# agiger/GPR

Measured on AMD Instinct MI355X. Metric: GP fits/sec (kernel build + Cholesky + solve), N=16384 d=32 fp64, higher is better.
Workload: dtype f64

## Files before the change

### gpr_amd/csrc/gprx_api.cpp

```cpp
#include <hip/hip_runtime.h>
#include <rccl/rccl.h>

#include <algorithm>
#include <climits>
#include <chrono>
#include <cmath>
#include <cstdlib>
#include <cstring>
#include <limits>
#include <memory>
#include <mutex>
#include <string>
#include <type_traits>
#include <vector>

#include "gprx_dist.h"
#include "gprx_internal.h"
#include "../../include/gprx_dev.h"

namespace gprx {

template <typename T>
void launch_pair_kernel(const KCanon<T>& K, const T* Xa, const T* Xb, int64_t q, int d, T* out, hipStream_t s);
template <typename T>
// ... 771 lines not shown
    } else if (!direct_build && pairs_mma_supported<T>(K, 1)) {
        const int64_t kf = pairs_feature_cols<T>(K, M->d);
        M->featU.ensure(sizeof(T) * np * kf);
        M->featV.ensure(sizeof(T) * np * kf);
        launch_pair_features<T>(K, M->X.as<T>(), n, M->d, M->X.as<T>(), false, M->featU.as<T>(), np, s,
                                M->flag.as<int>());
        launch_pair_features<T>(K, M->X.as<T>(), n, M->d, M->X.as<T>(), true, M->featV.as<T>(), np, s);
        const KCanon<T>* kdev = M->kfit.put(K, s);
        if (!separate_build && potrf_uses_tiles())
            tb = pairs_tile_build<T>(K, kdev, M->featU.as<T>(), M->featV.as<T>(), np, M->d, n, sigma2,
                                     M->flag.as<int>());
        if (!tb.mode)
            launch_kbuild_mma<T>(K, kdev, M->featU.as<T>(), M->featV.as<T>(), np, M->d, M->A.as<T>(),
                                 ld, n, sigma2, M->flag.as<int>(), s);
        launch_aug_rows<T>(M->Y.as<T>(), n, M->m, M->A.as<T>(), ld, np, mp, s);
    } else {
        launch_kbuild<T>(K, M->X.as<T>(), M->tab.as<T>(), n, M->X.as<T>(), M->tab.as<T>(), n, M->d, M->A.as<T>(), ld,
                         np, true, sigma2, M->flag.as<int>(), s);
        launch_aug_rows<T>(M->Y.as<T>(), n, M->m, M->A.as<T>(), ld, np, mp, s);
    }
    GPRX_HIP(hipEventRecord(ctx->ev[1], s));
    if (tb.mode || want_inv) {
        potrf_tiles<T>(M->A.as<T>(), ld, np, ld, M->Linv.as<T>(), M->info.as<int>(), ctx->ex, tb.mode ? &tb : nullptr,
                       want_inv ? (int)(np / GT) : 0);
    } else {
        potrf_auto<T>(M->A.as<T>(), ld, np, ld, M->Linv.as<T>(), M->info.as<int>(), ctx->ex);
    }
    GPRX_HIP(hipEventRecord(ctx->ev[2], s));
    launch_fit_reductions<T>(M->A.as<T>(), ld, n, np, M->m, M->red.as<double>(), s);
    launch_backsolve_chain<T>(M->A.as<T>(), ld, np, M->m, M->Linv.as<T>(), M->alpha.as<T>(), M->info.as<int>(), ctx->ex,
                              s);
    if (want_inv) {
        M->C.ensure(sizeof(T) * np * np);
        const T* U = M->A.as<T>() + np + mp;
        launch_gemm_nt_kskip<T>(M->C.as<T>(), np, U, ld, U, ld, np, np, np, s);
    }
    GPRX_HIP(hipEventRecord(ctx->ev[3], s));
    M->hstat.ensure(4 * sizeof(double));
    volatile double* hs = static_cast<double*>(M->hstat.p);
    launch_fit_status_gather(M->flag.as<int>(), M->info.as<int>(), M->red.as<double>(), M->hstat.dev, s);
    GPRX_HIP(hipStreamSynchronize(s));
    GPRX_HIP(hipGetLastError());
    int hflag = 0, hinfo = 0;
    double hred[2] = {hs[2], hs[3]};
    hflag = reinterpret_cast<volatile int*>(hs)[0];
    hinfo = reinterpret_cast<volatile int*>(hs + 1)[0];
    M->fitted = false;
// ... 2062 lines not shown
```

### gpr_amd/csrc/gprx_dev.cpp

```cpp
#include <hip/hip_runtime.h>

#include <algorithm>
#include <climits>
#include <cstring>
#include <string>
#include <vector>

#include "../../include/gprx_dev.h"
#include "gprx_internal.h"

namespace gprx {
template <typename T>
void launch_gemm_nt(T* C, int64_t ldc, const T* A, int64_t lda, const T* B, int64_t ldb, int64_t M, int64_t N,
                    int64_t K, T alpha, T beta, bool lower, hipStream_t s);
template <typename T>
void launch_diag_public(T* Akk, int64_t ld, T* Lk, int* info, int64_t col0, hipStream_t s, int ph = 3);
template <typename T>
void launch_diag_prof(T* Akk, int64_t ld, T* Lk, int* info, long long* prof, hipStream_t s);
namespace pt {
template <typename T>
void launch_diag_bench(int variant, T* A, int64_t ld, T* Linv, int* info, long long* prof, int reps, hipStream_t s);
}
}

// ... 284 lines not shown
}
extern "C" int64_t gprx_dev_bs_trace(int64_t* times, int64_t max_blocks) {
    try {
        return gprx::bs_trace_copy((long long*)times, max_blocks);
    } catch (const Error& e) {
        std::fprintf(stderr, "gprx_dev_bs_trace: %s\n", e.msg.c_str());
        return -1;
    }
}
extern "C" int64_t gprx_dev_pt_trace(int32_t* tasks, int64_t* times, int64_t max) {
    try {
        return gprx::pt_trace_copy(tasks, (long long*)times, max);
    } catch (const gprx::Error& e) {
        std::fprintf(stderr, "gprx_dev_pt_trace: %s\n", e.msg.c_str());
        return -1;
    }
}
extern "C" int32_t gprx_dev_pt_debug(int32_t* out, int32_t max_wg) { return gprx::pt_debug_snapshot(out, max_wg); }

extern "C" gprx_status gprx_dev_schedule(int32_t nc, int32_t nr, int32_t P, int32_t build, double* est_us,
                                         int64_t* ntasks) {
    try {
        const int64_t n = potrf_tiles_schedule_stats(nc, nr, P, (build & 1) != 0, est_us, (build & 2) ? nc : 0,
                                                     ((build >> 8) & 0xff) - 1, nullptr, 0, ((build >> 16) & 0xff) - 1);
        if (ntasks) *ntasks = n;
        return GPRX_OK;
    } catch (const Error& e) {
        std::fprintf(stderr, "gprx_dev_schedule: %s\n", e.msg.c_str());
        return e.st;
    }
}

extern "C" int64_t gprx_dev_schedule_list(int32_t nc, int32_t nr, int32_t P, int32_t build, int32_t* out,
                                          int64_t max) {
    try {
        return potrf_tiles_schedule_stats(nc, nr, P, (build & 1) != 0, nullptr, (build & 2) ? nc : 0,
                                          ((build >> 8) & 0xff) - 1, out, max, ((build >> 16) & 0xff) - 1);
    } catch (const Error& e) {
        std::fprintf(stderr, "gprx_dev_schedule_list: %s\n", e.msg.c_str());
        return -1;
    }
}

namespace gprx {
gprx_status gprx_dev_bench_impl(gprx_dtype dtype, int32_t what, int64_t M, int64_t N, int64_t K, int32_t iters,
                                double* ms, Exec* ex) {
    return dtype == GPRX_F64 ? bench_impl<double>(what, M, N, K, iters, ms, *ex)
                             : bench_impl<float>(what, M, N, K, iters, ms, *ex);
}
}

extern "C" gprx_status gprx_dev_fexp(gprx_ctx* ctx, const double* x, int64_t n, double* y) {
    (void)ctx;
    if (n <= 0) return GPRX_OK;
    double *dx = nullptr, *dy = nullptr;
    if (hipMalloc(&dx, sizeof(double) * n) != hipSuccess || hipMalloc(&dy, sizeof(double) * n) != hipSuccess)
        return GPRX_ERR_OOM;
    (void)hipMemcpy(dx, x, sizeof(double) * n, hipMemcpyHostToDevice);
    hipLaunchKernelGGL(dev_fexp_kernel, dim3((unsigned)((n + 255) / 256)), dim3(256), 0, 0, dx, n, dy);
    const hipError_t e = hipMemcpy(y, dy, sizeof(double) * n, hipMemcpyDeviceToHost);
// ... 53 lines not shown
```

### gpr_amd/csrc/gprx_internal.h

```cpp
#pragma once

#include <hip/hip_runtime.h>
#include <rccl/rccl.h>
#include <cstdint>
#include <cstdio>
#include <string>
#include <vector>

#include "../../include/gprx.h"

namespace gprx {

constexpr int MAX_LEAF = 8;
constexpr int MAX_TERM = 16;
constexpr int MAX_PER = 2;

enum LeafType { L_GAUSS = 1, L_GAUSS_EXP = 2, L_WHITE = 3, L_RQ = 4, L_PERIODIC = 5 };

template <typename T>
struct KLeaf {
    int type;
    int pslot;
    T c0, c1, c2;
    T p[3];
// ... 394 lines not shown
                         double* acc, hipStream_t s,
                         const uint64_t* ctab = nullptr);
template <typename T>
void launch_lml_grad_mma_cross(const KCanon<T>& K, const KCanon<T>* Kd, const T* Xa, int64_t na, const T* Xb,
                               int64_t nb, const T* center, int d, const T* FU, int64_t nfu, const T* FV, int64_t nfv,
                               T* GU, T* GV, const T* a, const T* b, const T* C, int64_t ldc, double* part, double* acc,
                               hipStream_t s);
template <typename T>
void launch_lml_grad_cross(const KCanon<T>& K, const T* Xa, const T* tabA, int64_t na, const T* Xb, const T* tabB,
                           int64_t nb, int d, const T* a, const T* b, const T* C, int64_t ldc, double* acc,
                           hipStream_t s);
template <typename T>
void launch_sparse_resid(const T* A, int64_t lda, int64_t n, int64_t M, const T* u, const T* y, T alpha, T* out,
                         hipStream_t s);
template <typename T>
void launch_sq_sum(const T* y, int64_t n, double* out, hipStream_t s);
template <typename T>
void launch_sub(const T* X, const T* Y, T* Z, int64_t e, hipStream_t s);
template <typename T>
TileBuild<T> pairs_tile_build(const KCanon<T>& K, const KCanon<T>* Kd, const T* FU, const T* FV, int64_t nf, int d,
                              int64_t n, T sigma2, int* flag);
template <typename T>
void potrf_tiles(T* A, int64_t ld, int64_t np, int64_t nrows, T* Linv, int* info, Exec& ex,
                 const TileBuild<T>* build = nullptr, int ni = 0, bool build_only = false);
template <typename T>
void launch_gemm_nt_kskip(T* C, int64_t ldc, const T* A, int64_t lda, const T* B, int64_t ldb, int64_t M, int64_t N,
                          int64_t K, hipStream_t s);
template <typename T>
void potrf_auto(T* A, int64_t ld, int64_t np, int64_t nrows, T* Linv, int* info, Exec& ex);
bool potrf_uses_tiles();
int64_t potrf_tiles_schedule_stats(int nc, int nr, int P, bool build, double* est_us, int ni = 0, int ratio = -1,
                                   int32_t* list_out = nullptr, int64_t list_max = 0, int pair = -1);
template <typename T>
void launch_gemm_nt(T* C, int64_t ldc, const T* A, int64_t lda, const T* B, int64_t ldb, int64_t M, int64_t N,
                    int64_t K, T alpha, T beta, bool lower, hipStream_t s);
template <typename T>
void launch_gemm_nt_splitk(T* C, int64_t ldc, int64_t cstride, const T* A, int64_t lda, const T* B, int64_t ldb,
                           int64_t M, int64_t N, int64_t K, int P, T alpha, bool lower, hipStream_t s);

template <typename T>
void launch_syrk_splitk(T* C, int64_t ldc, int64_t cstride, const T* A, int64_t lda, int64_t M, int64_t N, int64_t K,
                        int P, T alpha, hipStream_t s);
template <typename T>
bool launch_gemm_tall(T* C, int64_t ldc, const T* A, int64_t lda, const T* B, int64_t ldb, int64_t M, int64_t N,
                      int64_t K, T alpha, T beta, hipStream_t s);

template <typename T>
void launch_backsolve(const T* A, int64_t ld, int64_t np, int m, const T* Linv, T* z, T* alpha, hipStream_t s);

constexpr long long CHAIN_TLIMIT_TICKS = 400000000LL;

struct BlockTrace {
    long long* dev = nullptr;
    int n = 0;
    long long* ensure(int nb) {
// ... 61 lines not shown
```

### gpr_amd/csrc/k_mma.h

```cpp
#pragma once
#include "gprx_internal.h"
#include "k_handoff.h"

namespace gprx {
namespace mm {

constexpr int NT = 512;
constexpr int PAD = 16;

enum { T_DIAGX = 0, T_TRSM = 1, T_UPD = 2, T_BUILD = 3, T_TPART = 4, T_UPD2 = 5 };
enum { C_TICKET = 0, C_ERR = 1, C_NCTL = 16 };

typedef double d4_t __attribute__((ext_vector_type(4)));
typedef float f4_t __attribute__((ext_vector_type(4)));
typedef double d2_t __attribute__((ext_vector_type(2)));

template <typename T>
struct Mfma;
template <>
struct Mfma<double> {
    typedef d4_t acc_t;
    typedef d2_t vec_t;
    static constexpr int VEC = 2;
    __device__ static inline acc_t mma(double a, double b, acc_t c) {
// ... 384 lines not shown
            const int kr = kq * 4 + lk;
            fa[r] = a[S::at(kr, 16 * w + lr)];
#pragma unroll
            for (int g = G0; g < 8; g++) fb[r][g] = b[S::at(kr, 16 * g + lr)];
        };
        frag(0, 0);
#pragma unroll
        for (int kq = 0; kq < BK / 4; kq++) {
            if (kq + 1 < BK / 4) frag(kq + 1, (kq + 1) & 1);
            __builtin_amdgcn_sched_barrier(0);
#pragma unroll
            for (int g = G0; g < 8; g++) acc[g >> 2][g & 3] = Tr::mma(fb[kq & 1][g], fa[kq & 1], acc[g >> 2][g & 3]);
        }
    };
    static_assert(NST <= 8, "trirows: at most 8 stages");
    stage(std::integral_constant<int, 0>{});
    if constexpr (NST > 1) stage(std::integral_constant<int, (NST > 1 ? 1 : 0)>{});
    if constexpr (NST > 2) stage(std::integral_constant<int, (NST > 2 ? 2 : 0)>{});
    if constexpr (NST > 3) stage(std::integral_constant<int, (NST > 3 ? 3 : 0)>{});
    if constexpr (NST > 4) stage(std::integral_constant<int, (NST > 4 ? 4 : 0)>{});
    if constexpr (NST > 5) stage(std::integral_constant<int, (NST > 5 ? 5 : 0)>{});
    if constexpr (NST > 6) stage(std::integral_constant<int, (NST > 6 ? 6 : 0)>{});
    if constexpr (NST > 7) stage(std::integral_constant<int, (NST > 7 ? 7 : 0)>{});
}

template <typename T>
constexpr size_t tall_lds() {
    return sizeof(T) * 2 * 3 * Stage<T>::GRP * Stage<T>::SRP;
}
template <typename T, int MID = 1>
__device__ __forceinline__ void tile_mma_tall(typename Mfma<T>::acc_t (&acc)[4][4], const T* __restrict__ A,
                                              int64_t lda, const T* __restrict__ B, int64_t ldb, int K, T* smem,
                                              const int t, const T* __restrict__ Csub = nullptr, int64_t ldc = 0) {
    typedef Mfma<T> Tr;
    typedef Stage<T> S;
    constexpr int BK = BkOf<T>::v;
    static_assert(S::ROT == 0, "tall tile: unrotated staging");
    constexpr int GR3 = 3 * S::GRP, IPW3 = GR3 / 8, STG3 = GR3 * S::SRP;
    static_assert(GR3 % 8 == 0, "tall tile: whole DMA instructions per wave");
    const int lane = t & 63, w = t >> 6;
    const int wr = w & 3, wc = w >> 2, lr = lane & 15, lk = lane >> 4;
    const int lcol = lane / S::LPC, lrow = S::src_row(lane);
    auto issue = [&](int st) {
        T* buf = smem + (st & 1) * STG3;
#pragma unroll
        for (int u = 0; u < IPW3; u++) {
// ... 203 lines not shown
```

### gpr_amd/csrc/k_ptiles.hip

```cpp
#include "gprx_dist.h"
#include "gprx_internal.h"
#include "k_handoff.h"
#include "k_pairs.h"

#include <algorithm>
#include <climits>
#include <cstring>
#include <cstdlib>
#include <functional>
#include <map>
#include <mutex>
#include <queue>
#include <tuple>

namespace gprx {

namespace pt {

using namespace mm;
using ho::ld_agent;
using ho::ld_sys;
using ho::ld_uni;
using ho::local_sync;
using ho::publish;
// ... 50 lines not shown
}

#ifndef GPRX_TRSM_ROWS
#define GPRX_TRSM_ROWS 1
#endif
template <typename T>
__device__ __forceinline__ void tile_trsm(T* C, int64_t ldc, const T* A, int64_t lda,
                                          const T* __restrict__ B, int64_t ldb, T* smem, const int t) {
    if constexpr (!GPRX_TRSM_ROWS) {
        tile_gemm<T, false, 1, GPRX_SHORT_FEED>(C, ldc, A, lda, B, ldb, GT, false, smem, t, true);
    } else {
        typedef Mfma<T> Tr;
        const int lane = t & 63, w = t >> 6, lr = lane & 15, lk = lane >> 4;
        typename Tr::acc_t acc[2][4];
        mm::tile_mma_trirows<T>(acc, A, lda, B, ldb, smem, t);
#pragma unroll
        for (int x = 0; x < 2; x++)
#pragma unroll
            for (int y = 0; y < 4; y++)
#pragma unroll
                for (int reg = 0; reg < 4; reg++)
                    st_sc1(C + (int64_t)(16 * (4 * x + y) + Tr::orow(lk, reg)) * ldc + 16 * w + lr, acc[x][y][reg]);
    }
}

template <typename T>
__device__ __forceinline__ void tile_gemm_tall(T* __restrict__ C, int64_t ldc, const T* __restrict__ A, int64_t lda,
                                               const T* __restrict__ B, int64_t ldb, int K, T* smem, const int t) {
    typedef Mfma<T> Tr;
    typedef typename Tr::acc_t acc_t;
    const int lane = t & 63, w = t >> 6;
    const int wr = w & 3, wc = w >> 2, lr = lane & 15, lk = lane >> 4;
    acc_t acc[4][4];
    mm::tile_mma_tall<T, 1>(acc, A, lda, B, ldb, K, smem, t, C, ldc);
#pragma unroll
    for (int x = 0; x < 4; x++)
#pragma unroll
        for (int reg = 0; reg < 4; reg++) {
            T* ccol = C + (int64_t)(64 * wc + 16 * x + Tr::orow(lk, reg)) * ldc;
#pragma unroll
            for (int y = 0; y < 4; y++) st_sc1(ccol + 64 * wr + 16 * y + lr, -acc[x][y][reg]);
        }
}

constexpr int SPL = DB + 4;
constexpr int SIL = DB + 2;
// ... 945 lines not shown
template <typename T>
struct Args {
    T* A;
    int64_t ld;
    T* Linv;
    const int4* tasks;
    int ntasks;
    int nc;
    int nv;
    int* ctl;
    int* lcnt;
    int* ver;
    int* info;
    long long tlimit;
    int* dbg;
    int variant;
    long long* trace;
    long long* xt;
    const TileBuild<T>* tb;
    const PtDist<T>* dist;
    int split;
    T* pbuf;
    int* tflag;
};


constexpr int DIST_TO_REC = 132;
__device__ __forceinline__ void dist_note_timeout(int* rec, int kind, int type, int i, int j, int b0nb, int detail,
                                                  int seen) {
    if (!rec) return;
    if (__hip_atomic_fetch_add(rec, 0, __ATOMIC_RELAXED, __HIP_MEMORY_SCOPE_AGENT) != 0) return;
    if (atomicCAS(rec, 0, kind) != 0) return;
    rec[1] = type;
    rec[2] = i;
    rec[3] = j;
    rec[4] = b0nb;
    rec[5] = detail;
    rec[6] = seen;
}

template <typename T>
__device__ __forceinline__ T* dist_tile(T* A, const PtDist<T>& D, int i, int j) {
    const int li = __builtin_amdgcn_readfirstlane(D.loc[i]);
    int col = j;
    if (i > D.nc) {
        const int aa = i - D.nc - 1;
        col = (j < D.nc) ? j - aa : D.nc - aa + (j - D.nc - 1);
// ... 1001 lines not shown
                    dist_push(Akm, D, cm & ~first, owin, dist_f_tile() + (int64_t)k * D.nc + (k - 1), tid, tix, tgv);
                if (ok) dist_push(a.Linv + (int64_t)k * DB * DB, D, all & ~first, olinv, dist_f_linv(D.nr, D.nc) + k, tid);
            }
            if (!ok) break;
        } else {
        T* Ci = a.A + (int64_t)i * GT;
        constexpr bool fused_ts = std::is_same<T, double>::value && DIAG_LA;
        if (type == T_TPART) {
            if constexpr (SPLIT_CODE)
                (void)tpart_task<T, false>(tpc, Ci + (int64_t)(i - 1) * GT * ld, Ci + (int64_t)i * GT * ld, ld,
                                           a.Linv + (int64_t)(i - 1) * DB * DB, i, j, smem, s_ok, tid,
                                           tp_linv_form() ? nullptr
                                                          : a.A + (int64_t)(i - 1) * GT + (int64_t)(i - 1) * GT * ld);
        } else if (type == T_BUILD) {
            const TileBuild<T>& b = *a.tb;
            const bool bad = pr::build_tile_sum<T, 1, true>(b.Kd, b.FU, b.FV, b.nf, b.Kr, b.Kp, b.hd, a.A, ld, b.n,
                                                            b.sigma2, (int64_t)i * GT, (int64_t)j * GT, smem, tid);
            if (__builtin_amdgcn_readfirstlane(__any(bad))) atomicOr(a.tb->flag, 1);
            publish(a.ver + (int64_t)i * a.nv + j, 0, false);
        } else if (type == T_UPD) {
            const int64_t oa = (a.variant & 64) ? 0 : (int64_t)i * GT + (int64_t)b0 * GT * ld;
            const int64_t ob = (a.variant & 64) ? GT : (int64_t)j * GT + (int64_t)b0 * GT * ld;
            const int64_t lop = (a.variant & 128) ? 0 : ld;
            if (!(a.variant & 2))
                tile_gemm<T, true>(Ci + (int64_t)j * GT * ld, ld, a.A + oa, lop, a.A + ob, lop, nb * GT, i == j, smem,
                                   tid);
            publish(a.ver + (int64_t)i * a.nv + j, b0 + nb, false);
        } else if (type == T_UPD2) {
            if (!(a.variant & 2))
                tile_gemm_tall<T>(Ci + (int64_t)j * GT * ld, ld, a.A + (int64_t)i * GT + (int64_t)b0 * GT * ld, ld,
                                  a.A + (int64_t)j * GT + (int64_t)b0 * GT * ld, ld, nb * GT, smem, tid);
            publish2(a.ver + (int64_t)i * a.nv + j, a.ver + (int64_t)(i + 1) * a.nv + j, b0 + nb);
        } else if (type == T_TRSM) {
            T* Cik = Ci + (int64_t)j * GT * ld;
            if (!(a.variant & 1))
                tile_trsm<T>(Cik, ld, Cik, ld, a.Linv + (int64_t)j * DB * DB, DB, smem, tid);
            publish(a.lcnt + i, j + 1, false);
        } else {
            const int k = i;
            T* Akk = Ci + (int64_t)k * GT * ld;
            long long dt[4] = {0, 0, 0, 0};
            if (SPLIT_CODE && k > 0 && a.split) {
                if constexpr (fused_ts) (void)diagx_split<T>(tpc, k, smem, s_ok, tid);
                else (void)diagx_split_wait<T>(tpc, k, s_ok);
                if (a.trace) dt[0] = dt[1] = wall_clock64();
            } else if (fused_ts && k > 0) {
                T* Akm = Ci + (int64_t)(k - 1) * GT * ld;
                dt[0] = diagx_ts<T>(Akm, Akk, ld, a.Linv + (int64_t)(k - 1) * DB * DB, a.lcnt + k, k, smem, tid,
                                    a.trace != nullptr);
// ... 27 lines not shown
            tp[3] = (long long)blockIdx.x | (((long long)__builtin_amdgcn_s_memtime() - tc1) << 16);
        }
    }
    dbg_mark(a.dbg, -1, 9, 0, 0);
    if (wv == 0 && ld_agent(a.ctl + C_ERR)) atomicMin(a.info, -1);
}

struct Cost {
    double k128 = 17.1;
    double ovh = 6.5;
    double trsm = 16.0;
    double diagx = 70.0;
    double diag0 = 40.0;
    double early = 31.0;
    double diagf = 0.97;
    double build = 28.0;
    double tpart = 11.5, tpart_c = 0.0;
    double diagx_s = 44.0, early_s = 2.0;
    double tpart_prog = 2.5;
    bool prog = false;
    int np = 4;
    double tall = 0.975;
    int pair_nbmin = 1, pair_tail = 0;
};

static void order_tparts(std::vector<int4>& list) {
    std::map<int, std::vector<int>> pos;
    for (size_t q = 0; q < list.size(); q++)
        if ((list[q].x & 0xff) == T_TPART) pos[list[q].y].push_back((int)q);
    for (auto& kv : pos) {
        std::vector<int>& v = kv.second;
        std::sort(v.begin(), v.end());
        for (size_t u = 0; u < v.size(); u++) list[v[u]].z = (int)v.size() - 1 - (int)u;
    }
}

struct Task {
    int type, i, j, b0, nb;
    double dur;
    std::vector<int> succ, esucc;
    int ndep = 0;
    double bl = 0;
};

struct Schedule {
    std::vector<int4> list;
// ... 14 lines not shown
                if (p == W && b % W) continue;
                const int end = b + p;
                if (end > e - near || p > ratio * (e - end)) continue;
                break;
            }
            out.push_back({s + b, p});
            b += p;
        }
        return;
    }
    int hb = std::max(0, std::min(W * ((j - s) / W), e));
    hb -= hb % W;
    int b = 0;
    for (; b + W <= hb; b += W) out.push_back({s + b, W});
    for (int p = W / 2; p >= 1; p /= 2)
        if (b + p <= e - near) {
            out.push_back({s + b, p});
            b += p;
        }
    for (; b < e; b++) out.push_back({s + b, 1});
}

static Schedule make_schedule(int nc, int nr, int W, int near, int P, const Cost& cm0, bool build, int ni = 0,
                              int ratio = 0, bool split = false, int tail = 0, int pair = 0) {
    Cost cm = cm0;
    if (split) cm.early = cm.early_s;
    const int nr0 = nr - ni;
    auto start_of = [&](int i) { return i >= nr0 ? i - nr0 : 0; };
    static const bool id_pair = [] {
        const char* e = std::getenv("GPRX_PT_IDPAIR");
        return !(e && std::atoi(e) == 0);
    }();
    const bool ident_even = id_pair && pair > 0 && ni > 1;
    static const bool id_tail = [] {
        const char* e = std::getenv("GPRX_PT_IDTAIL");
        return !(e && std::atoi(e) == 0);
    }();
    auto cstart = [&](int i) {
        const int a = start_of(i);
        return (ident_even && i >= nr0) ? a - (a & 1) : a;
    };
    auto pair_role = [&](int i, int j) {
        if (pair <= 0) return 0;
        if (i >= nr0) {
            const int a = i - nr0;
            if (!ident_even) return 0;
            if ((a & 1) == 0) return a + 1 < ni ? 1 : 0;
            return 2;
        }
        const int r0 = j + pair;
        if (i >= r0 && (i - r0) % 2 == 0 && i + 1 < nr0) return 1;
        if (i - 1 >= r0 && (i - 1 - r0) % 2 == 0) return 2;
        return 0;
    };
    std::vector<Task> tasks;
    tasks.reserve((size_t)nr * nc * 2);
    auto add = [&](int type, int i, int j, int b0, int nb, double dur) {
        Task tk;
        tk.type = type;
        tk.i = i;
        tk.j = j;
        tk.b0 = b0;
        tk.nb = nb;
        tk.dur = dur;
        tasks.push_back(std::move(tk));
        return (int)tasks.size() - 1;
    };
    std::vector<int> diagx(nc, -1);
    std::vector<int> trsm((size_t)nr * nc, -1);
    std::vector<int> last_upd((size_t)nr * nc, -1);
    std::vector<std::vector<int>> deps, edeps;
    auto dep = [&](int tsk, int on, bool early = false) {
        if (on < 0) return;
        auto& d = early ? edeps : deps;
        if ((int)d.size() <= tsk) d.resize(tsk + 1);
// ... 51 lines not shown
            if (k < start_of(i)) continue;
            const int id = add(T_TRSM, i, k, 0, 0, cm.trsm);
            trsm[(size_t)i * nc + k] = id;
            dep(id, diagx[k]);
            dep(id, last_upd[(size_t)i * nc + k]);
        }
        if (k + 1 < nc) make_diagx(k + 1);
        for (const Chunk& c : by_last[k]) {
            const bool pairable = c.nb >= cm.pair_nbmin && (c.j < nc - cm.pair_tail || (c.i >= nr0 && id_tail));
            const int role = pairable ? pair_role(c.i, c.j) : 0;
            if (role == 2) continue;
            if (role == 1) {
                const int id = add(T_UPD2, c.i, c.j, c.b0, c.nb, cm.ovh + 2.0 * c.nb * cm.k128 * cm.tall);
                bool e1, e2, e3;
                for (int r = c.i; r <= c.i + 1; r++) dep(id, last_upd[(size_t)r * nc + c.j]);
                const int p1 = prodL(c.i, k, e1), p3 = prodL(c.i + 1, k, e3), p2 = prodL(c.j, k, e2);
                dep(id, p1, e1);
                dep(id, p3, e3);
                dep(id, p2, e2);
                last_upd[(size_t)c.i * nc + c.j] = id;
                last_upd[(size_t)(c.i + 1) * nc + c.j] = id;
                continue;
            }
            const double dur = cm.ovh + c.nb * cm.k128 * (c.i == c.j ? cm.diagf : 1.0);
            const int id = add(T_UPD, c.i, c.j, c.b0, c.nb, dur);
            dep(id, last_upd[(size_t)c.i * nc + c.j]);
            bool e1, e2;
            const int p1 = prodL(c.i, k, e1), p2 = prodL(c.j, k, e2);
            dep(id, p1, e1);
            dep(id, p2, e2);
            last_upd[(size_t)c.i * nc + c.j] = id;
        }
    }
    const int nt = (int)tasks.size();
    deps.resize(nt);
    edeps.resize(nt);
    for (int id = 0; id < nt; id++) {
        auto& d = deps[id];
        auto& ed = edeps[id];
        std::sort(d.begin(), d.end());
        d.erase(std::unique(d.begin(), d.end()), d.end());
        std::sort(ed.begin(), ed.end());
        ed.erase(std::unique(ed.begin(), ed.end()), ed.end());
        for (int on : d) {
            if (on >= id) throw Error{GPRX_ERR_ARG, "potrf tile schedule: producer created after consumer"};
            tasks[on].succ.push_back(id);
        }
// ... 304 lines not shown
        now = f.first;
        if (f.second < 0) {
            for (int s2 : tasks[-1 - f.second].esucc)
                if (--indeg[s2] == 0) make_ready(s2);
            continue;
        }
        if (rank_of[f.second] >= 0) freew[rank_of[f.second]]++;
        for (int s2 : tasks[f.second].succ)
            if (--indeg[s2] == 0) make_ready(s2);
    }
    S.est_us = now;
    S.W = W;
    if (split)
        for (auto& l : S.lists) order_tparts(l);
    return S;
}

struct Params {
    int W = 64, near = -1;
    int ratio = -1;
    int split = 1;
    int tail = 0;
    int pair = -1;
    Cost cm;
    int near_for(int nc) const { return near >= 0 ? near : (nc <= 64 ? 1 : 0); }
    Params() {
        if (const char* e = std::getenv("GPRX_PT_W")) W = std::max(1, std::atoi(e));
        if (const char* e = std::getenv("GPRX_PT_NEAR")) near = std::max(0, std::atoi(e));
        if (const char* e = std::getenv("GPRX_PT_RATIO")) ratio = std::max(0, std::atoi(e));
        if (const char* e = std::getenv("GPRX_PT_DIAGX_US")) cm.diagx = std::atof(e);
        if (const char* e = std::getenv("GPRX_PT_TRSM_US")) cm.trsm = std::atof(e);
        if (const char* e = std::getenv("GPRX_PT_K128_US")) cm.k128 = std::atof(e);
        if (const char* e = std::getenv("GPRX_PT_OVH_US")) cm.ovh = std::atof(e);
        if (const char* e = std::getenv("GPRX_PT_BUILD_US")) cm.build = std::atof(e);
        if (const char* e = std::getenv("GPRX_PT_SPLIT")) split = std::atoi(e);
        if (const char* e = std::getenv("GPRX_PT_TAIL")) tail = std::atoi(e);
        if (const char* e = std::getenv("GPRX_PT_PAIR")) pair = std::atoi(e);
        if (const char* e = std::getenv("GPRX_PT_TALL")) cm.tall = std::atof(e);
        if (const char* e = std::getenv("GPRX_PT_PAIR_NBMIN")) cm.pair_nbmin = std::max(1, std::atoi(e));
        if (const char* e = std::getenv("GPRX_PT_PAIR_TAIL")) cm.pair_tail = std::max(0, std::atoi(e));
        if (const char* e = std::getenv("GPRX_PT_TPART_US")) cm.tpart = std::atof(e);
        if (const char* e = std::getenv("GPRX_PT_DIAGXS_US")) cm.diagx_s = std::atof(e);
        if (const char* e = std::getenv("GPRX_PT_TPARTP_US")) cm.tpart_prog = std::atof(e);
    }
    Cost cost(bool f64) const {
        Cost c = cm;
        c.prog = f64 && DIAG_LA && !tp_linv_form();
        c.np = tp_parts(f64 && DIAG_LA);
        return c;
    }
};
static const Params& params() {
    static Params p;
    return p;
}

static const int kRatios[] = {0, 8, 4, 2};
static const int kTails[] = {0, 16, 32};
struct PairRule {
    int pair, nbmin, tail;
};
static PairRule default_pair(bool f64) { return f64 ? PairRule{4, 4, 32} : PairRule{2, 4, 16}; }
static Schedule best_schedule(int nc, int nr, const Params& pr, int P, bool build, int ni, bool split, bool f64) {
    Cost cm = pr.cost(f64);
    const PairRule pd = default_pair(f64);
    if (!std::getenv("GPRX_PT_PAIR_NBMIN")) cm.pair_nbmin = pd.nbmin;
    if (!std::getenv("GPRX_PT_PAIR_TAIL")) cm.pair_tail = ni > 0 ? 0 : pd.tail;
    Schedule best;
    bool have = false;
    const int want = pr.pair >= 0 ? pr.pair : pd.pair;
    for (int pq : {want}) {
        auto consider = [&](Schedule&& S) {
            if (!have || S.est_us < best.est_us * 0.995) {
                best = std::move(S);
                have = true;
            }
        };
        if (pr.ratio >= 0) {
            consider(make_schedule(nc, nr, pr.W, pr.near_for(nc), P, cm, build, ni, pr.ratio, split, pr.tail, pq));
            continue;
        }
        for (int r : kRatios)
            for (int tl : kTails) {
                if ((r == 0 && tl) || (tl && tl >= nc)) continue;
                consider(make_schedule(nc, nr, pr.W, pr.near_for(nc), P, cm, build, ni, r, split, tl, pq));
            }
    }
    return best;
}

static bool split_for(bool f64) { (void)f64; return SPLIT_CODE && params().split != 0; }
static bool split_for(bool f64, int P) { return P >= tp_parts(f64 && DIAG_LA) && split_for(f64); }

}

struct PtState {
    struct Dev {
        int4* list = nullptr;
        int64_t n = 0;
        double est_us = 0;
        bool ident_even = false;
        std::vector<int4> host;
    };
    std::map<std::tuple<int, int, bool, int, bool, int>, Dev> sched;
    int* ctr = nullptr;
    void* pbuf = nullptr;
    size_t ctr_ints = 0;
    int ncu = 0;
// ... 53 lines not shown
}

__global__ void pt_init_identity_counters(int* __restrict__ lcnt, int* __restrict__ ver, int nc, int nr0, int ni,
                                          int even) {
    const int a = blockIdx.x, j = threadIdx.x;
    if (a >= ni) return;
    if (j == 0) lcnt[nr0 + a] = a;
    const int v = even ? a - (a & 1) : a;
    for (int c = j; c < nc; c += blockDim.x) ver[(int64_t)(nr0 + a) * nc + c] = v;
}

template <typename T>
__global__ void pt_init_identity_rows(T* __restrict__ A, int64_t ld, int64_t row0, int64_t nid, int64_t ncol,
                                      int even) {
    const int64_t r = (int64_t)blockIdx.x * blockDim.x + threadIdx.x;
    const int64_t c = blockIdx.y;
    const int64_t rb = r / GT, c0 = (even ? rb - (rb & 1) : rb) * GT;
    if (r >= nid || c >= ncol || c < c0) return;
    A[row0 + r + c * ld] = (r == c) ? T(1) : T(0);
}

template <typename T>
void potrf_tiles(T* A, int64_t ld, int64_t np, int64_t nrows, T* Linv, int* info, Exec& ex, const TileBuild<T>* build,
                 int ni, bool build_only) {
    using namespace pt;
    if (!ex.pt) ex.pt = new PtState();
    PtState& st = *ex.pt;
    if (st.ncu == 0) {
        int dev = 0;
        GPRX_HIP(hipGetDevice(&dev));
        hipDeviceProp_t prop;
        GPRX_HIP(hipGetDeviceProperties(&prop, dev));
        st.ncu = prop.multiProcessorCount;
    }
    GPRX_REQUIRE(np % DB == 0 && nrows % GT == 0 && nrows >= np, GPRX_ERR_ARG, "potrf_tiles: bad sizes");
    const int nc = (int)(np / DB), nr = (int)(nrows / GT);
    const bool fused = build && build->mode != 0;
    GPRX_REQUIRE(ni >= 0 && ni <= nr - nc, GPRX_ERR_ARG, "potrf_tiles: bad identity row blocks");
    GPRX_REQUIRE(!build_only || fused, GPRX_ERR_ARG, "potrf_tiles: build_only needs a fused build");
    const bool split = split_for(std::is_same<T, double>::value, st.ncu);
    auto key = std::make_tuple(nc, nr, fused, build_only ? -1 : ni, split, (int)sizeof(T));
    auto it = st.sched.find(key);
    if (it == st.sched.end()) {
        const Params& pr = params();
        Schedule S;
        if (build_only) {
            for (int i = 0; i < nc; i++)
                for (int j = 0; j <= i; j++) S.list.push_back(make_int4(T_BUILD, i, j, 0));
        } else {
            S = best_schedule(nc, nr, pr, st.ncu, fused, ni, split, std::is_same<T, double>::value);
        }
        PtState::Dev d;
        d.n = (int64_t)S.list.size();
        d.est_us = S.est_us;
        d.ident_even = S.ident_even;
        GPRX_HIP(hipMalloc(&d.list, sizeof(int4) * std::max<int64_t>(1, d.n)));
        GPRX_HIP(hipMemcpy(d.list, S.list.data(), sizeof(int4) * d.n, hipMemcpyHostToDevice));
        d.host = S.list;
        it = st.sched.emplace(key, d).first;
    }
    const PtState::Dev& sd = it->second;
    const size_t need = (size_t)C_NCTL + nr + (size_t)nr * nc + TP_STRIDE * (size_t)nc;
    if (st.ctr_ints < need) {
        if (st.ctr) GPRX_HIP(hipFree(st.ctr));
        st.ctr = nullptr;
        GPRX_HIP(hipMalloc(&st.ctr, sizeof(int) * need));
        st.ctr_ints = need;
    }
    hipStream_t s = ex.s0;
    {
        const int64_t v0 = fused ? (int64_t)C_NCTL + nr : 0, v1 = fused ? v0 + (int64_t)nc * nc : 0;
        hipLaunchKernelGGL(pt_init_counters, dim3((unsigned)((need + 255) / 256)), dim3(256), 0, s, st.ctr,
                           (int64_t)need, v0, v1);
// ... 3 lines not shown
        hipLaunchKernelGGL(pt_init_identity_counters, dim3((unsigned)ni), dim3(128), 0, s, st.ctr + C_NCTL,
                           st.ctr + C_NCTL + nr, nc, nr - ni, ni, sd.ident_even ? 1 : 0);
        hipLaunchKernelGGL(pt_init_identity_rows<T>, dim3((unsigned)((ni * (int64_t)GT + 255) / 256), (unsigned)np),
                           dim3(256), 0, s, A, ld, (int64_t)(nr - ni) * GT, (int64_t)ni * GT, np, sd.ident_even ? 1 : 0);
    }
    Args<T> a;
    a.A = A;
    a.ld = ld;
    a.Linv = Linv;
    a.tasks = sd.list;
    a.ntasks = (int)sd.n;
    a.nc = nc;
    a.nv = nc;
    a.ctl = st.ctr;
    a.lcnt = st.ctr + C_NCTL;
    a.ver = st.ctr + C_NCTL + nr;
    a.info = info;
    a.tb = nullptr;
    a.dist = nullptr;
    a.split = split ? 1 : 0;
    a.tflag = st.ctr + C_NCTL + nr + (size_t)nr * nc;
    if (split && !st.pbuf) GPRX_HIP(hipMalloc(&st.pbuf, sizeof(T) * 4 * DB * DB));
    a.pbuf = static_cast<T*>(st.pbuf);
    if (fused) {
        GPRX_REQUIRE(build->nf == np, GPRX_ERR_ARG, "potrf_tiles: build features must have np rows");
        if (!st.tb) GPRX_HIP(hipMalloc(&st.tb, sizeof(TileBuild<double>)));
        const unsigned char* tbb = reinterpret_cast<const unsigned char*>(build);
        if (st.tb_last.size() != sizeof(TileBuild<T>) || std::memcmp(st.tb_last.data(), tbb, sizeof(TileBuild<T>)) != 0) {
            GPRX_HIP(hipMemcpyAsync(st.tb, build, sizeof(TileBuild<T>), hipMemcpyHostToDevice, s));
            st.tb_last.assign(tbb, tbb + sizeof(TileBuild<T>));
        }
        a.tb = reinterpret_cast<const TileBuild<T>*>(st.tb);
    }
    a.dbg = nullptr;
    a.trace = nullptr;
    a.xt = nullptr;
    static const bool tracing = std::getenv("GPRX_PT_TRACE") != nullptr;
    if (tracing) {
        if (st.trace_n + 7 * st.trace_nc < sd.n + 7 * nc) {
            if (st.trace) GPRX_HIP(hipFree(st.trace));
            GPRX_HIP(hipMalloc(&st.trace, sizeof(long long) * 4 * (sd.n + 7 * nc)));
        }
        st.trace_n = sd.n;
        st.trace_nc = nc;
        a.trace = st.trace;
        a.xt = st.trace + 4 * (sd.n + 2 * nc);
// ... 47 lines not shown
    using namespace pt;
    Args<T> a;
    std::memset(&a, 0, sizeof(a));
    a.A = L.A;
    a.ld = DB;
    a.Linv = L.Linv;
    a.tasks = L.list;
    a.ntasks = L.ntasks;
    a.nc = L.nc;
    a.nv = L.nci;
    a.ctl = L.ctr;
    a.lcnt = L.ctr + C_NCTL;
    a.ver = L.ctr + C_NCTL + L.nr;
    a.info = L.info;
    a.tlimit = L.tlimit;
    a.tb = L.tb_dev;
    a.dist = L.dist_dev;
    a.dbg = L.dbg;
    a.trace = L.trace;
    a.xt = nullptr;
    a.split = L.split;
    a.pbuf = L.pbuf;
    a.tflag = L.tflag;
    auto lds_of = [](size_t b) { return std::max<size_t>(b, 96 * 1024); };
    const size_t lds = lds_of(pt_lds_total<T>());
    static bool attr = false;
    if (!attr) {
        GPRX_HIP(hipFuncSetAttribute((const void*)potrf_tiles_kernel<double, true>,
                                     hipFuncAttributeMaxDynamicSharedMemorySize, (int)lds_of(pt_lds_total<double>())));
        GPRX_HIP(hipFuncSetAttribute((const void*)potrf_tiles_kernel<float, true>,
                                     hipFuncAttributeMaxDynamicSharedMemorySize, (int)lds_of(pt_lds_total<float>())));
        attr = true;
    }
    hipLaunchKernelGGL((potrf_tiles_kernel<T, true>), dim3((unsigned)L.P), dim3(NT), lds, L.s, a);
    GPRX_HIP(hipGetLastError());
}
template void potrf_tiles_dist_launch<double>(const DistLaunch<double>&);
template void potrf_tiles_dist_launch<float>(const DistLaunch<float>&);

int64_t potrf_tiles_schedule_stats(int nc, int nr, int P, bool build, double* est_us, int ni, int ratio,
                                   int32_t* list_out, int64_t list_max, int pair) {
    if (nc < 1 || nr < nc || P < 1 || ni < 0 || ni > nr - nc)
        throw Error{GPRX_ERR_ARG, "potrf tile schedule: need nc >= 1, nr >= nc + ni, P >= 1"};
    pt::Params pr = pt::params();
    if (pair >= 0) pr.pair = pair;
    const bool split = pt::split_for(true, P);
    pt::Schedule S = ratio >= 0 ? pt::make_schedule(nc, nr, pr.W, pr.near_for(nc), P, pr.cost(true), build, ni, ratio, split,
                                                    pr.tail, pr.pair > 0 ? pr.pair : 0)
                                : pt::best_schedule(nc, nr, pr, P, build, ni, split, true);
    if (est_us) *est_us = S.est_us;
    if (list_out)
        for (int64_t q = 0; q < (int64_t)S.list.size() && q < list_max; q++) {
            const int4 t = S.list[q];
            list_out[4 * q] = t.x, list_out[4 * q + 1] = t.y, list_out[4 * q + 2] = t.z, list_out[4 * q + 3] = t.w;
        }
    return S.ntasks;
}

bool potrf_split_for(bool f64, int P) { return pt::split_for(f64, P); }

template void potrf_tiles<double>(double*, int64_t, int64_t, int64_t, double*, int*, Exec&, const TileBuild<double>*,
                                  int, bool);
template void potrf_tiles<float>(float*, int64_t, int64_t, int64_t, float*, int*, Exec&, const TileBuild<float>*, int,
                                 bool);

}
```

Before: 39.78.

## Use narrow 16-row GEMM for label row block in tiled Cholesky

When the appended label/RHS row block carries at most 16 live rows (few targets), the trailing update of that block uses a new 16-row MFMA GEMM instead of the full-tile GEMM, which skips work on padding rows. The scheduler gets a narrow mode that gives these label tasks their own cost and keeps them out of the paired-row update grouping, so it can place them better. This adds a second kernel path and a schedule-cache key variant, and relies on the unused rows of the label block staying unread.

New measurement: 40.35 (median of 6 runs). +1.4%, better.

```diff
diff --git a/gpr_amd/csrc/gprx_api.cpp b/gpr_amd/csrc/gprx_api.cpp
--- a/gpr_amd/csrc/gprx_api.cpp
+++ b/gpr_amd/csrc/gprx_api.cpp
@@ -817,7 +817,7 @@
     GPRX_HIP(hipEventRecord(ctx->ev[1], s));
     if (tb.mode || want_inv) {
         potrf_tiles<T>(M->A.as<T>(), ld, np, ld, M->Linv.as<T>(), M->info.as<int>(), ctx->ex, tb.mode ? &tb : nullptr,
-                       want_inv ? (int)(np / GT) : 0);
+                       want_inv ? (int)(np / GT) : 0, false, mp == GT ? M->m : GT);
     } else {
         potrf_auto<T>(M->A.as<T>(), ld, np, ld, M->Linv.as<T>(), M->info.as<int>(), ctx->ex);
     }
diff --git a/gpr_amd/csrc/gprx_dev.cpp b/gpr_amd/csrc/gprx_dev.cpp
--- a/gpr_amd/csrc/gprx_dev.cpp
+++ b/gpr_amd/csrc/gprx_dev.cpp
@@ -330,7 +330,8 @@
                                          int64_t* ntasks) {
     try {
         const int64_t n = potrf_tiles_schedule_stats(nc, nr, P, (build & 1) != 0, est_us, (build & 2) ? nc : 0,
-                                                     ((build >> 8) & 0xff) - 1, nullptr, 0, ((build >> 16) & 0xff) - 1);
+                                                     ((build >> 8) & 0xff) - 1, nullptr, 0, ((build >> 16) & 0xff) - 1,
+                                                     (build & 4) != 0);
         if (ntasks) *ntasks = n;
         return GPRX_OK;
     } catch (const Error& e) {
@@ -343,7 +344,8 @@
                                           int64_t max) {
     try {
         return potrf_tiles_schedule_stats(nc, nr, P, (build & 1) != 0, nullptr, (build & 2) ? nc : 0,
-                                          ((build >> 8) & 0xff) - 1, out, max, ((build >> 16) & 0xff) - 1);
+                                          ((build >> 8) & 0xff) - 1, out, max, ((build >> 16) & 0xff) - 1,
+                                          (build & 4) != 0);
     } catch (const Error& e) {
         std::fprintf(stderr, "gprx_dev_schedule_list: %s\n", e.msg.c_str());
         return -1;
diff --git a/gpr_amd/csrc/gprx_internal.h b/gpr_amd/csrc/gprx_internal.h
--- a/gpr_amd/csrc/gprx_internal.h
+++ b/gpr_amd/csrc/gprx_internal.h
@@ -440,7 +440,7 @@
                               int64_t n, T sigma2, int* flag);
 template <typename T>
 void potrf_tiles(T* A, int64_t ld, int64_t np, int64_t nrows, T* Linv, int* info, Exec& ex,
-                 const TileBuild<T>* build = nullptr, int ni = 0, bool build_only = false);
+                 const TileBuild<T>* build = nullptr, int ni = 0, bool build_only = false, int lab_live = GT);
 template <typename T>
 void launch_gemm_nt_kskip(T* C, int64_t ldc, const T* A, int64_t lda, const T* B, int64_t ldb, int64_t M, int64_t N,
                           int64_t K, hipStream_t s);
@@ -448,7 +448,8 @@
 void potrf_auto(T* A, int64_t ld, int64_t np, int64_t nrows, T* Linv, int* info, Exec& ex);
 bool potrf_uses_tiles();
 int64_t potrf_tiles_schedule_stats(int nc, int nr, int P, bool build, double* est_us, int ni = 0, int ratio = -1,
-                                   int32_t* list_out = nullptr, int64_t list_max = 0, int pair = -1);
+                                   int32_t* list_out = nullptr, int64_t list_max = 0, int pair = -1,
+                                   bool narrow = false);
 template <typename T>
 void launch_gemm_nt(T* C, int64_t ldc, const T* A, int64_t lda, const T* B, int64_t ldb, int64_t M, int64_t N,
                     int64_t K, T alpha, T beta, bool lower, hipStream_t s);
diff --git a/gpr_amd/csrc/k_mma.h b/gpr_amd/csrc/k_mma.h
--- a/gpr_amd/csrc/k_mma.h
+++ b/gpr_amd/csrc/k_mma.h
@@ -430,6 +430,75 @@
     if constexpr (NST > 5) stage(std::integral_constant<int, (NST > 5 ? 5 : 0)>{});
     if constexpr (NST > 6) stage(std::integral_constant<int, (NST > 6 ? 6 : 0)>{});
     if constexpr (NST > 7) stage(std::integral_constant<int, (NST > 7 ? 7 : 0)>{});
+}
+
+template <typename T>
+__device__ __forceinline__ void tile_mma_rows16(typename Mfma<T>::acc_t& acc, const T* __restrict__ A, int64_t lda,
+                                                const T* __restrict__ B, int64_t ldb, int K, T* smem, const int t) {
+    typedef Mfma<T> Tr;
+    typedef typename Tr::acc_t acc_t;
+    constexpr int BK = BkOf<T>::v;
+    typedef Stage<T, BK> S;
+    const int lane = t & 63, w = t >> 6;
+    const int lr = lane & 15, lk = lane >> 4;
+    const int lcol = lane / S::LPC, lrow = S::src_row(lane);
+    auto issue = [&](int st) {
+        T* buf = smem + (st % S::NB) * S::STG;
+#pragma unroll
+        for (int u = 0; u < S::IPW; u++) {
+            const int g = w * S::IPW + u;
+            const bool isB = g >= S::GRP;
+            const int gg = isB ? g - S::GRP : g;
+            const int64_t col = (int64_t)st * BK + gg * S::CPI + lcol;
+            const T* src = isB ? (B + lrow + col * ldb) : (A + lrow + col * lda);
+            __builtin_amdgcn_global_load_lds((const void*)src,
+                                             (__attribute__((address_space(3))) void*)(buf + g * S::SRP), 16, 0, 0);
+        }
+    };
+    acc = acc_t{0};
+    const int nst = __builtin_amdgcn_readfirstlane(K) / BK;
+#pragma unroll
+    for (int p = 0; p < S::AH; p++)
+        if (p < nst) issue(p);
+#pragma nounroll
+    for (int st = 0; st < nst; st++) {
+        const int ahead = nst - 1 - st;
+        if (S::AH >= 3 && ahead >= 2) wait_vm<(S::AH >= 3 ? 2 : 0) * S::IPW>();
+        else if (S::AH >= 2 && ahead >= 1) wait_vm<S::IPW>();
+        else wait_vm<0>();
+        asm volatile("s_waitcnt lgkmcnt(0)" ::: "memory");
+        __builtin_amdgcn_s_barrier();
+        if (st + S::AH < nst) issue(st + S::AH);
+        const T* a = smem + (st % S::NB) * S::STG;
+        const T* b = a + S::GRP * S::SRP;
+        constexpr bool PAIRED = sizeof(T) == 4 && BK >= 32 && S::CPI == 2 && S::ROT == 0;
+        if constexpr (PAIRED) {
+            T pa[BK / 8][2], pb[BK / 8][2];
+#pragma unroll
+            for (int j = 0; j < BK / 8; j++) {
+                const T* ac = a + (4 * j + lk) * S::SRP;
+                const T* bc = b + (4 * j + lk) * S::SRP;
+#pragma unroll
+                for (int h = 0; h < 2; h++) {
+                    pa[j][h] = ac[h * GT + lr];
+                    pb[j][h] = bc[h * GT + 16 * w + lr];
+                }
+            }
+#pragma unroll
+            for (int j = 0; j < BK / 8; j++)
+#pragma unroll
+                for (int h = 0; h < 2; h++) acc = Tr::mma(pb[j][h], pa[j][h], acc);
+        } else {
+            T fa[BK / 4], fb[BK / 4];
+#pragma unroll
+            for (int kq = 0; kq < BK / 4; kq++) {
+                fa[kq] = a[S::at(kq * 4 + lk, lr)];
+                fb[kq] = b[S::at(kq * 4 + lk, 16 * w + lr)];
+            }
+#pragma unroll
+            for (int kq = 0; kq < BK / 4; kq++) acc = Tr::mma(fb[kq], fa[kq], acc);
+        }
+    }
 }
 
 template <typename T>
diff --git a/gpr_amd/csrc/k_ptiles.hip b/gpr_amd/csrc/k_ptiles.hip
--- a/gpr_amd/csrc/k_ptiles.hip
+++ b/gpr_amd/csrc/k_ptiles.hip
@@ -96,6 +96,20 @@
                 for (int reg = 0; reg < 4; reg++)
                     st_sc1(C + (int64_t)(16 * (4 * x + y) + Tr::orow(lk, reg)) * ldc + 16 * w + lr, acc[x][y][reg]);
     }
+}
+
+template <typename T>
+__device__ __forceinline__ void tile_gemm_rows16(T* __restrict__ C, int64_t ldc, const T* __restrict__ A, int64_t lda,
+                                                 const T* __restrict__ B, int64_t ldb, int K, T* smem, const int t) {
+    typedef Mfma<T> Tr;
+    const int lane = t & 63, w = t >> 6, lr = lane & 15, lk = lane >> 4;
+    T cv[4];
+#pragma unroll
+    for (int reg = 0; reg < 4; reg++) cv[reg] = C[(int64_t)(16 * w + Tr::orow(lk, reg)) * ldc + lr];
+    typename Tr::acc_t acc;
+    mm::tile_mma_rows16<T>(acc, A, lda, B, ldb, K, smem, t);
+#pragma unroll
+    for (int reg = 0; reg < 4; reg++) st_sc1(C + (int64_t)(16 * w + Tr::orow(lk, reg)) * ldc + lr, cv[reg] - acc[reg]);
 }
 
 template <typename T>
@@ -1087,7 +1101,9 @@
     int split;
     T* pbuf;
     int* tflag;
+    int lab_rows;
 };
+constexpr int LAB_NARROW = 16;
 
 
 constexpr int DIST_TO_REC = 132;
@@ -2135,9 +2151,13 @@
             const int64_t oa = (a.variant & 64) ? 0 : (int64_t)i * GT + (int64_t)b0 * GT * ld;
             const int64_t ob = (a.variant & 64) ? GT : (int64_t)j * GT + (int64_t)b0 * GT * ld;
             const int64_t lop = (a.variant & 128) ? 0 : ld;
-            if (!(a.variant & 2))
+            if (a.variant & 2) {
+            } else if (i == a.nc && a.lab_rows <= LAB_NARROW) {
+                tile_gemm_rows16<T>(Ci + (int64_t)j * GT * ld, ld, a.A + oa, lop, a.A + ob, lop, nb * GT, smem, tid);
+            } else {
                 tile_gemm<T, true>(Ci + (int64_t)j * GT * ld, ld, a.A + oa, lop, a.A + ob, lop, nb * GT, i == j, smem,
                                    tid);
+            }
             publish(a.ver + (int64_t)i * a.nv + j, b0 + nb, false);
         } else if (type == T_UPD2) {
             if (!(a.variant & 2))
@@ -2211,6 +2231,7 @@
     int np = 4;
     double tall = 0.975;
     int pair_nbmin = 1, pair_tail = 0;
+    double klab = 4.3;
 };
 
 static void order_tparts(std::vector<int4>& list) {
@@ -2271,10 +2292,12 @@
 }
 
 static Schedule make_schedule(int nc, int nr, int W, int near, int P, const Cost& cm0, bool build, int ni = 0,
-                              int ratio = 0, bool split = false, int tail = 0, int pair = 0) {
+                              int ratio = 0, bool split = false, int tail = 0, int pair = 0, bool narrow = false) {
     Cost cm = cm0;
     if (split) cm.early = cm.early_s;
     const int nr0 = nr - ni;
+    narrow = narrow && nr0 == nc + 1;
+    const int pend = narrow ? nc : nr0;
     auto start_of = [&](int i) { return i >= nr0 ? i - nr0 : 0; };
     static const bool id_pair = [] {
         const char* e = std::getenv("GPRX_PT_IDPAIR");
@@ -2298,8 +2321,8 @@
             return 2;
         }
         const int r0 = j + pair;
-        if (i >= r0 && (i - r0) % 2 == 0 && i + 1 < nr0) return 1;
-        if (i - 1 >= r0 && (i - 1 - r0) % 2 == 0) return 2;
+        if (i >= r0 && (i - r0) % 2 == 0 && i + 1 < pend) return 1;
+        if (i - 1 >= r0 && (i - 1 - r0) % 2 == 0 && i < pend) return 2;
         return 0;
     };
     std::vector<Task> tasks;
@@ -2397,7 +2420,8 @@
                 last_upd[(size_t)(c.i + 1) * nc + c.j] = id;
                 continue;
             }
-            const double dur = cm.ovh + c.nb * cm.k128 * (c.i == c.j ? cm.diagf : 1.0);
+            const bool lab = narrow && c.i == nc && cm.klab >= 0;
+            const double dur = cm.ovh + c.nb * (lab ? cm.klab : cm.k128 * (c.i == c.j ? cm.diagf : 1.0));
             const int id = add(T_UPD, c.i, c.j, c.b0, c.nb, dur);
             dep(id, last_upd[(size_t)c.i * nc + c.j]);
             bool e1, e2;
@@ -2748,6 +2772,7 @@
     int split = 1;
     int tail = 0;
     int pair = -1;
+    int label = 1;
     Cost cm;
     int near_for(int nc) const { return near >= 0 ? near : (nc <= 64 ? 1 : 0); }
     Params() {
@@ -2768,6 +2793,8 @@
         if (const char* e = std::getenv("GPRX_PT_TPART_US")) cm.tpart = std::atof(e);
         if (const char* e = std::getenv("GPRX_PT_DIAGXS_US")) cm.diagx_s = std::atof(e);
         if (const char* e = std::getenv("GPRX_PT_TPARTP_US")) cm.tpart_prog = std::atof(e);
+        if (const char* e = std::getenv("GPRX_PT_KLAB_US")) cm.klab = std::atof(e);
+        if (const char* e = std::getenv("GPRX_PT_LABEL")) label = std::atoi(e);
     }
     Cost cost(bool f64) const {
         Cost c = cm;
@@ -2787,7 +2814,8 @@
     int pair, nbmin, tail;
 };
 static PairRule default_pair(bool f64) { return f64 ? PairRule{4, 4, 32} : PairRule{2, 4, 16}; }
-static Schedule best_schedule(int nc, int nr, const Params& pr, int P, bool build, int ni, bool split, bool f64) {
+static Schedule best_schedule(int nc, int nr, const Params& pr, int P, bool build, int ni, bool split, bool f64,
+                              bool narrow = false) {
     Cost cm = pr.cost(f64);
     const PairRule pd = default_pair(f64);
     if (!std::getenv("GPRX_PT_PAIR_NBMIN")) cm.pair_nbmin = pd.nbmin;
@@ -2803,13 +2831,13 @@
             }
         };
         if (pr.ratio >= 0) {
-            consider(make_schedule(nc, nr, pr.W, pr.near_for(nc), P, cm, build, ni, pr.ratio, split, pr.tail, pq));
+            consider(make_schedule(nc, nr, pr.W, pr.near_for(nc), P, cm, build, ni, pr.ratio, split, pr.tail, pq, narrow));
             continue;
         }
         for (int r : kRatios)
             for (int tl : kTails) {
                 if ((r == 0 && tl) || (tl && tl >= nc)) continue;
-                consider(make_schedule(nc, nr, pr.W, pr.near_for(nc), P, cm, build, ni, r, split, tl, pq));
+                consider(make_schedule(nc, nr, pr.W, pr.near_for(nc), P, cm, build, ni, r, split, tl, pq, narrow));
             }
     }
     return best;
@@ -2909,7 +2937,7 @@
 
 template <typename T>
 void potrf_tiles(T* A, int64_t ld, int64_t np, int64_t nrows, T* Linv, int* info, Exec& ex, const TileBuild<T>* build,
-                 int ni, bool build_only) {
+                 int ni, bool build_only, int lab_live) {
     using namespace pt;
     if (!ex.pt) ex.pt = new PtState();
     PtState& st = *ex.pt;
@@ -2926,7 +2954,8 @@
     GPRX_REQUIRE(ni >= 0 && ni <= nr - nc, GPRX_ERR_ARG, "potrf_tiles: bad identity row blocks");
     GPRX_REQUIRE(!build_only || fused, GPRX_ERR_ARG, "potrf_tiles: build_only needs a fused build");
     const bool split = split_for(std::is_same<T, double>::value, st.ncu);
-    auto key = std::make_tuple(nc, nr, fused, build_only ? -1 : ni, split, (int)sizeof(T));
+    const bool narrow = !build_only && lab_live <= LAB_NARROW && nr - ni == nc + 1 && params().label != 0;
+    auto key = std::make_tuple(nc, nr, fused, build_only ? -1 : ni, split, (int)sizeof(T) | (narrow ? 256 : 0));
     auto it = st.sched.find(key);
     if (it == st.sched.end()) {
         const Params& pr = params();
@@ -2935,7 +2964,7 @@
             for (int i = 0; i < nc; i++)
                 for (int j = 0; j <= i; j++) S.list.push_back(make_int4(T_BUILD, i, j, 0));
         } else {
-            S = best_schedule(nc, nr, pr, st.ncu, fused, ni, split, std::is_same<T, double>::value);
+            S = best_schedule(nc, nr, pr, st.ncu, fused, ni, split, std::is_same<T, double>::value, narrow);
         }
         PtState::Dev d;
         d.n = (int64_t)S.list.size();
@@ -2985,6 +3014,7 @@
     a.tflag = st.ctr + C_NCTL + nr + (size_t)nr * nc;
     if (split && !st.pbuf) GPRX_HIP(hipMalloc(&st.pbuf, sizeof(T) * 4 * DB * DB));
     a.pbuf = static_cast<T*>(st.pbuf);
+    a.lab_rows = narrow ? lab_live : GT;
     if (fused) {
         GPRX_REQUIRE(build->nf == np, GPRX_ERR_ARG, "potrf_tiles: build features must have np rows");
         if (!st.tb) GPRX_HIP(hipMalloc(&st.tb, sizeof(TileBuild<double>)));
@@ -3078,6 +3108,7 @@
     a.split = L.split;
     a.pbuf = L.pbuf;
     a.tflag = L.tflag;
+    a.lab_rows = GT;
     auto lds_of = [](size_t b) { return std::max<size_t>(b, 96 * 1024); };
     const size_t lds = lds_of(pt_lds_total<T>());
     static bool attr = false;
@@ -3095,15 +3126,15 @@
 template void potrf_tiles_dist_launch<float>(const DistLaunch<float>&);
 
 int64_t potrf_tiles_schedule_stats(int nc, int nr, int P, bool build, double* est_us, int ni, int ratio,
-                                   int32_t* list_out, int64_t list_max, int pair) {
+                                   int32_t* list_out, int64_t list_max, int pair, bool narrow) {
     if (nc < 1 || nr < nc || P < 1 || ni < 0 || ni > nr - nc)
         throw Error{GPRX_ERR_ARG, "potrf tile schedule: need nc >= 1, nr >= nc + ni, P >= 1"};
     pt::Params pr = pt::params();
     if (pair >= 0) pr.pair = pair;
     const bool split = pt::split_for(true, P);
     pt::Schedule S = ratio >= 0 ? pt::make_schedule(nc, nr, pr.W, pr.near_for(nc), P, pr.cost(true), build, ni, ratio, split,
-                                                    pr.tail, pr.pair > 0 ? pr.pair : 0)
-                                : pt::best_schedule(nc, nr, pr, P, build, ni, split, true);
+                                                    pr.tail, pr.pair > 0 ? pr.pair : 0, narrow)
+                                : pt::best_schedule(nc, nr, pr, P, build, ni, split, true, narrow);
     if (est_us) *est_us = S.est_us;
     if (list_out)
         for (int64_t q = 0; q < (int64_t)S.list.size() && q < list_max; q++) {
@@ -3116,8 +3147,8 @@
 bool potrf_split_for(bool f64, int P) { return pt::split_for(f64, P); }
 
 template void potrf_tiles<double>(double*, int64_t, int64_t, int64_t, double*, int*, Exec&, const TileBuild<double>*,
-                                  int, bool);
+                                  int, bool, int);
 template void potrf_tiles<float>(float*, int64_t, int64_t, int64_t, float*, int*, Exec&, const TileBuild<float>*, int,
-                                 bool);
-
-}
+                                 bool, int);
+
+}
```
